# furkanyesiler/acoss

Measured on AMD Instinct MI355X. Metric: track-pairs/sec on N x N Serra09 Qmax (HPCP, T=2000), higher is better.
Workload: dtype f32

## Files before the change

acoss_amd/_lib.py:

```python
import ctypes
import os

import numpy as np

_HERE = os.path.dirname(os.path.abspath(__file__))
LIB_PATH = os.environ.get("ACX_LIB") or os.path.join(_HERE, "csrc", "libacx.so")

ACX_OK = 0
ACX_ERR_INVALID = -1
ACX_ERR_HIP = -2
ACX_ERR_NOMEM = -3
ACX_ERR_STATE = -4
ACX_ERR_SHORT = -5
ACX_ERR_UNSUPPORTED = -6

EXPORTS = [
    "acx_abi_version", "acx_create", "acx_destroy", "acx_last_error", "acx_set_scratch_limit",
    "acx_upload_pool", "acx_serra09_default_params", "acx_serra09_pairs", "acx_serra09_debug_pair",
    "acx_serra09_embed_len", "acx_profile_enable", "acx_profile_reset", "acx_profile_count",
    "acx_profile_get", "acx_debug_sqrt", "acx_debug_ef_sqrt", "acx_upload_pool_f64", "acx_simple_pairs",
    "acx_ef_upload_pool", "acx_earlyfusion_pairs", "acx_ef_debug_pair", "acx_sw_binary",
    "acx_chenfusion_pairs", "acx_csm_binary_sw", "acx_upload_raw_pool", "acx_download_pool",
    "acx_simple_upload_raw_pool", "acx_download_pool_f64", "acx_snf_fuse", "acx_qmax_binary",
    "acx_ef_block_features", "acx_ef_upload_raw_pool", "acx_snf_fuse_dists", "acx_grid_plan", "acx_pool_lengths", "acx_grid_run", "acx_grid_scatter", "acx_pair_grid",
    "acx_set_nonfinite_policy", "acx_nonfinite_zeroed", "acx_ef_pool_begin", "acx_ef_pool_tracks", "acx_ef_pool_end",
    "acx_set_ef_gemm", "acx_hip_versions",
    "acx_dev_alloc", "acx_dev_free", "acx_dev_read", "acx_dev_sync",
    "acx_comm_id", "acx_comm_init", "acx_comm_destroy", "acx_grid_allgather", "acx_pair_grid_ranks", "acx_set_ef_fuse",
    "acx_device_info", "acx_ef_debug_pairs",
    "acx_ftm2d_default_params", "acx_ftm2d_pool_begin", "acx_ftm2d_pool_tracks", "acx_ftm2d_pool_end",
    "acx_ftm2d_upload_shingles", "acx_ftm2d_download_shingles", "acx_ftm2d_debug_track", "acx_ftm2d_pairs",
    "acx_rank_columns", "acx_topk_rows",
    "acx_query_scores", "acx_query_topk", "acx_query_ranks", "acx_query_topk_lists",
    "acx_serra09_debug_bits", "acx_serra09_plan", "acx_serra09_family_name", "acx_serra09_fast_tail", "acx_serra09_fast_tail_launches",
    "acx_pool_append", "acx_pool_append_raw", "acx_pool_append_f64", "acx_ef_pool_append", "acx_ftm2d_append_shingles",
    "acx_pool_truncate",
    "acx_serra09_align", "acx_qmax_locate_binary",
    "acx_serra09_align_paths", "acx_qmax_path_binary",
    "acx_chenfusion_align", "acx_chenfusion_align_paths", "acx_dmax_locate_binary", "acx_dmax_path_binary",
    "acx_ef_debug_bits", "acx_csm_debug_bits", "acx_sw_bits_binary",
    "acx_ef_align", "acx_sw_align_binary",
    "acx_simple_profile",
    "acx_snf_debug_stages", "acx_snf_debug_update",
    "acx_ef_crossfusion_pairs", "acx_ef_crossfusion_debug", "acx_crossfusion_matrices", "acx_xsel_binary_sw",
    "acx_ef_download_pool",
]
ABI_VERSION = 4
COMM_ID_BYTES = 128

# ... 146 lines not shown
    L.acx_upload_pool.argtypes = [vp, fp, lp, ctypes.c_int32, ctypes.c_int32]
    L.acx_upload_raw_pool.argtypes = [vp, fp, lp, ctypes.c_int32, ctypes.c_int32, ctypes.c_int32, lp]
    L.acx_download_pool.argtypes = [vp, fp, ctypes.c_int64]
    L.acx_serra09_default_params.restype = None
    L.acx_serra09_default_params.argtypes = [pp]
    L.acx_serra09_pairs.argtypes = [vp, ip, ctypes.c_int64, pp, fp]
    L.acx_chenfusion_pairs.argtypes = [vp, ip, ctypes.c_int64, pp, fp]
    L.acx_serra09_debug_pair.argtypes = [vp, ctypes.c_int32, ctypes.c_int32, pp, fp, fp, fp, fp, fp, ip, fp, ip]
    L.acx_serra09_debug_bits.argtypes = [vp, ip, ctypes.c_int64, pp, fp, ctypes.POINTER(ctypes.c_uint8), ctypes.POINTER(ctypes.c_int64)]
    L.acx_serra09_plan.argtypes = [lp, ctypes.c_int32, ip, ctypes.c_int64, pp, ctypes.c_int64, ctypes.POINTER(Serra09PlanRec)]
    L.acx_serra09_family_name.restype = ctypes.c_char_p
    L.acx_serra09_family_name.argtypes = [ctypes.c_int32, ctypes.c_int32]
    L.acx_serra09_fast_tail.argtypes = [pp, ctypes.c_int32, ctypes.c_int32, ctypes.c_int32]
    L.acx_serra09_fast_tail_launches.restype = ctypes.c_int64
    L.acx_serra09_fast_tail_launches.argtypes = []
    L.acx_serra09_embed_len.restype = ctypes.c_int32
    L.acx_serra09_embed_len.argtypes = [ctypes.c_int32, pp]
    L.acx_profile_enable.argtypes = [vp, ctypes.c_int]
    L.acx_profile_reset.argtypes = [vp]
    L.acx_profile_count.argtypes = [vp]
    L.acx_profile_get.argtypes = [vp, ctypes.c_int, ctypes.c_char_p, ctypes.c_int,
                                  ctypes.POINTER(ctypes.c_double), lp, lp]
    L.acx_debug_sqrt.argtypes = [vp, fp, ctypes.c_int64, fp]
    L.acx_debug_ef_sqrt.argtypes = [vp, fp, ctypes.c_int64, fp]
    dp = ctypes.POINTER(ctypes.c_double)
    L.acx_upload_pool_f64.argtypes = [vp, dp, lp, ctypes.c_int32, ctypes.c_int32]
    L.acx_simple_upload_raw_pool.argtypes = [vp, fp, lp, ctypes.c_int32, ctypes.c_int32, ctypes.c_int32, ctypes.c_int32,
                                             ctypes.c_int32, lp]
    L.acx_download_pool_f64.argtypes = [vp, dp, ctypes.c_int64]
    L.acx_simple_pairs.argtypes = [vp, ip, ctypes.c_int64, ctypes.c_int32, ctypes.c_int32, dp]
# ... 180 lines not shown


def serra09_fast_tail(n_cells, role, params=None, debug=False):
    L = load()
    params = params if params is not None else serra09_params()
    rc = L.acx_serra09_fast_tail(ctypes.byref(params), int(n_cells), int(role), int(bool(debug)))
    if rc < 0:
        raise ValueError("acx_serra09_fast_tail: bad argument")
    return bool(rc)


def serra09_fast_tail_launches():
    return int(load().acx_serra09_fast_tail_launches())


def serra09_family_name(family, m):
    name = load().acx_serra09_family_name(int(family), int(m))
    if name is None:
        raise ValueError("unknown Serra09 kernel family %r" % (family,))
    return name.decode()


def grid_scatter(lengths, spec, gathered, rank_stride, planes, mirror, first=0, count=-1):
    L = load()
    lengths = np.ascontiguousarray(lengths, dtype=np.int64)
    gathered = np.ascontiguousarray(gathered, dtype=np.float32)
    n = len(lengths)
    for P in planes:
        if P.dtype != np.float32 or P.shape != (n, n) or not P.flags["C_CONTIGUOUS"]:
            raise ValueError("grid_scatter: planes must be C-contiguous (N, N) float32")
# ... 968 lines not shown
```

acoss_amd/csrc/acx.hip:

```cpp
#include <hip/hip_runtime.h>

#include <chrono>
#include <dlfcn.h>
#include <rccl/rccl.h>

#include <algorithm>
#include <cmath>
#include <cstdio>
#include <cstdlib>
#include <cstring>
#include <string>
#include <vector>

#include "../../include/acx.h"
#include "serra09_kernels.hpp"
#include "serra09_long_kernels.hpp"
#include "serra09_locate_kernels.hpp"
#include "serra09_path_kernels.hpp"
#include "chen_align_kernels.hpp"
#include "prep_kernels.hpp"
#include "snf_kernels.hpp"
#include "ef_crossfusion_kernels.hpp"
#include "simple_kernels.hpp"
#include "simple_profile_kernels.hpp"
// ... 56 lines not shown

struct acx_ctx {
    int device = 0;
    hipStream_t stream = nullptr;
    hipStream_t qstream = nullptr;
    hipStream_t qstream2 = nullptr;
    hipEvent_t q2_done = nullptr;
    std::string err;
    DeviceBuffer<float> d_frames0;
    DeviceBuffer<int64_t> d_toff0;
    std::vector<int64_t> h_off0;
    int pool_tau = 0;
    DeviceBuffer<float> d_frames;
    DeviceBuffer<float> d_frot;
    DeviceBuffer<_Float16> d_fh;
    DeviceBuffer<float> d_normtab;
    DeviceBuffer<int64_t> d_noff;
    int normtab_m = 0, normtab_span = -1;
    std::vector<int64_t> h_noff;
    DeviceBuffer<int64_t> d_toff;
    DeviceBuffer<float> d_gch;
    std::vector<int64_t> h_off;
    const float *active_frames() const { return d_frames ? d_frames.get() : d_frames0.get(); }
    const int64_t *active_toff() const { return d_toff ? d_toff.get() : d_toff0.get(); }
    int32_t n_tracks = 0, dim = 0;
    DeviceBuffer<double> d_frames64;
    DeviceBuffer<int64_t> d_toff64;
    DeviceBuffer<double> d_prof64;
    DeviceBuffer<double> d_wn64;
    int wn64_L = 0;
// ... 205 lines not shown
    if (p.pct_mode < 0 || p.pct_mode > 3) return fail(c, ACX_ERR_INVALID, "serra09: pct_mode must be 0..3");
    if (p.oti_target != 0 && p.oti_target != 1) return fail(c, ACX_ERR_INVALID, "serra09: oti_target must be 0 or 1");
    if (!(p.gamma_o >= 0.0f) || !(p.gamma_e >= 0.0f)) return fail(c, ACX_ERR_INVALID, "serra09: gammas must be >= 0");
    if (p.arith != ACX_ARITH_EXACT && p.arith != ACX_ARITH_F16X2) return fail(c, ACX_ERR_INVALID, "serra09: arith must be ACX_ARITH_EXACT or ACX_ARITH_F16X2");
    if (p.arith == ACX_ARITH_F16X2 && p.m != 9) return fail(c, ACX_ERR_UNSUPPORTED, "serra09: the f16x2 Gram exists for the default stack size m = 9 only");
    return ACX_OK;
}

constexpr int64_t POOL_SLACK = 96;

bool launch_band(acx_ctx *c, int m, const PairDesc *dpd, const std::vector<PairDesc> &hpd, int b0, int B, int maxRows, int cls,
                 const acx_serra09_params &p, int role, int write_d2, int want_eps)
{
    const float *operands = p.arith == ACX_ARITH_F16X2 ? reinterpret_cast<const float *>(c->d_fh + POOL_SLACK * acx::FH) : c->d_frot + POOL_SLACK * acx::FROT;
    acx::BandLaunch L{c->stream, operands, c->active_toff(), c->d_normtab + POOL_SLACK, c->d_noff, c->d_scratch, c->d_thr,
                      c->d_bits, p.kappa, p.pct_mode, p.inclusive, p.oti_target, 0};
    const int family = acx::serra09_band_family(cls, m, p.arith);
    bool ok = true;
    for (const acx::Serra09Run &r : acx::serra09_fast_tail_runs(p, family, role, write_d2 != 0, want_eps != 0, c->d_bits != nullptr, hpd, b0, b0 + B)) {
        L.fast_tail = r.fast ? 1 : 0;
        ok = ok && acx::launch_band_kernel(L, m, dpd + (r.begin - b0), r.end - r.begin, maxRows, family, role, write_d2, want_eps, p.arith);
    }
    return ok;
}

template <int M>
void launch_normtab(acx_ctx *c, int maxM, int span, int first, int count)
{
    hipLaunchKernelGGL((acx::normtab_kernel<M>), dim3(count, (maxM + 255) / 256, acx::NBIN), dim3(256), 0, c->stream,
                       c->active_frames(), c->active_toff() + first, c->d_noff + first, c->d_normtab + POOL_SLACK, span);
}
// ... 12 lines not shown
        case 13: CALL(13); break; case 14: CALL(14); break; case 15: CALL(15); break; case 16: CALL(16); break; \
        default: handled = false;                                                                   \
    }
#endif

int ensure_tau(acx_ctx *c, int tau)
{
    if (c->pool_tau == tau) return ACX_OK;
    c->normtab_m = 0; c->normtab_span = -1;
    c->pool_tau = 0;
    c->fh_base_n = -1;
    ACX_HIP(c, c->d_frames.reset());
    ACX_HIP(c, c->d_toff.reset());
    ACX_HIP(c, c->d_frot.reset());
    ACX_HIP(c, c->d_fh.reset());
    ACX_HIP(c, c->d_normtab.reset());
    ACX_HIP(c, c->d_noff.reset());
    const int n = c->n_tracks;
    DeviceBuffer<float> frames, frot;
    DeviceBuffer<int64_t> toff;
    if (tau == 1) {
        c->h_off = c->h_off0;
    } else {
        c->h_off.assign((size_t)n + 1, 0);
        int maxT = 1;
        for (int t = 0; t < n; ++t) {
            const int64_t T = c->h_off0[t + 1] - c->h_off0[t];
            const int64_t Td = (T + tau - 1) / tau;
            c->h_off[t + 1] = c->h_off[t] + Td;
            maxT = std::max<int>(maxT, (int)Td);
// ... 62 lines not shown
    DeviceBuffer<_Float16> fh;
    const hipError_t e = fh.grow(halfs);
    if (e != hipSuccess) return fail(c, ACX_ERR_NOMEM, std::string("serra09: the f16 operand pool does not fit the device: ") + hipGetErrorString(e));
    ACX_HIP(c, hipMemsetAsync(fh, 0, sizeof(_Float16) * halfs, c->stream));
    if (total > 0) {
        hipLaunchKernelGGL(acx::rotpool_f16_kernel, dim3((unsigned)std::min<int64_t>((total * 12 + 255) / 256, 1 << 22)), dim3(256), 0, c->stream,
                           c->active_frames(), fh + POOL_SLACK * acx::FH, total);
        ACX_HIP(c, hipGetLastError());
    }
    ACX_HIP(c, hipStreamSynchronize(c->stream));
    c->d_fh = std::move(fh);
    c->fh_base_n = total > 0 ? c->n_tracks : -1;
    return ACX_OK;
}

int ensure_normtab(acx_ctx *c, const acx_serra09_params &p)
{
    const int span = p.embed_full ? (p.m - 1) : p.m;
    if (c->d_normtab && c->normtab_m == p.m && c->normtab_span == span) return ACX_OK;
    ACX_HIP(c, c->d_normtab.reset());
    ACX_HIP(c, c->d_noff.reset());
    c->normtab_m = 0; c->normtab_span = -1;
    std::vector<int64_t> &noff = c->h_noff;
    noff.assign((size_t)c->n_tracks + 1, 0);
    int64_t tot = 0;
    int maxM = 1;
    for (int t = 0; t < c->n_tracks; ++t) {
        noff[t] = tot;
        const int Me = std::max<int>(0, (int)(c->h_off[t + 1] - c->h_off[t]) - span);
        maxM = std::max(maxM, Me);
// ... 17 lines not shown
    c->normtab_span = span;
    return ACX_OK;
}

struct DebugOut {
    float *d2, *epsq, *epsr, *thrq, *thrr;
    int32_t *oti;
    int32_t *dims;
};

int64_t scratch_limit_bytes(const acx_ctx *c)
{
    if (c->scratch_limit > 0) return c->scratch_limit;
    const char *env = getenv("ACX_SCRATCH_GB");
    if (env && atof(env) > 0) return (int64_t)(atof(env) * (double)(1ull << 30));
    return (int64_t)(0.40 * (double)c->total_mem);
}

int collect_slot(acx_ctx *c, Serra09Slot &s, float *out, acx_alignment *al = nullptr)
{
    if (!s.busy) return ACX_OK;
    ACX_HIP(c, hipEventSynchronize(s.done));
    for (int k2 = 0; s.al && al && k2 < s.B; ++k2) al[s.k0 + s.perm[k2]] = s.h_al[(size_t)k2];
    for (int k2 = 0; !s.al && out && k2 < s.B; ++k2)
        for (int e = 0; e < s.w; ++e) out[(size_t)s.w * (s.k0 + s.perm[k2]) + e] = s.h_out[(size_t)s.w * k2 + e];
    s.busy = false;
    drain_profile(c);
    return ACX_OK;
}

struct DevDst {
// ... 265 lines not shown

    int64_t k0 = 0;
    for (int batch = 0; k0 < K; ++batch) {
        Serra09Slot &S = c->slot[batch & 1];
        if ((rc = collect_slot(c, S, out, al)) != ACX_OK) return rc;
        std::vector<PairDesc> &pd = S.pd;
        acx::Serra09Arena used;
        const int64_t k = acx::serra09_pack_batch(len, pairs, k0, K, p, dbg != nullptr, limit_floats, pd, used);
        if (k == k0) return fail(c, ACX_ERR_STATE, "serra09: the batch plan made no progress at pair " + std::to_string(k0));
        const int B = (int)pd.size();
        const acx::Serra09Sort srt = acx::serra09_sort_batch(pd, S.sorted, S.perm, p.m);
        const int *key_begin = srt.key_begin, *cls_begin = srt.cls_begin;
        const std::vector<int> &perm = S.perm;
        if (cls_begin[NC] > 0 && (rc = ensure_normtab(c, p)) != ACX_OK) return rc;
        if (cls_begin[NC] > 0 && p.arith == ACX_ARITH_F16X2 && (rc = ensure_f16pool(c)) != ACX_OK) return rc;
        if ((rc = ensure(c, c->d_scratch, (size_t)std::max<int64_t>(used.scratch, 1))) != ACX_OK) return rc;
        if ((rc = ensure(c, c->d_bits, (size_t)std::max<int64_t>(used.bits, 1))) != ACX_OK) return rc;
        if ((rc = ensure(c, c->d_thr, (size_t)used.thr + 64 * 32 + 16)) != ACX_OK) return rc;
        if ((rc = ensure(c, S.d_pd, (size_t)B)) != ACX_OK) return rc;
        if ((rc = ensure(c, S.d_out, (size_t)2 * B)) != ACX_OK) return rc;
        if ((rc = ensure(c, S.h_out, (size_t)2 * B)) != ACX_OK) return rc;
        ACX_HIP(c, hipMemcpyAsync(S.d_pd, pd.data(), sizeof(PairDesc) * B, hipMemcpyHostToDevice, c->stream));
        if (al) {
            int64_t seams = 0;
            S.seam_off.resize((size_t)B);
            for (int k2 = 0; k2 < B; ++k2) { S.seam_off[(size_t)k2] = seams; seams += acx::loc_seam_records(pd[k2].Mq, pd[k2].Mr, p.dp_start); }
            if ((rc = ensure(c, S.d_al, (size_t)B)) != ACX_OK) return rc;
            if ((rc = ensure(c, S.h_al, (size_t)B)) != ACX_OK) return rc;
            if ((rc = ensure(c, S.d_seam_off, (size_t)B)) != ACX_OK) return rc;
            if ((rc = ensure(c, c->d_seam, (size_t)std::max<int64_t>(seams, 1))) != ACX_OK) return rc;
// ... 701 lines not shown
#undef ACX_ROWSTAT
#undef ACX_FUSESEL
#undef ACX_FUSESEL_K
#undef ACX_SW
    if (host_timing)
        fprintf(stderr, "[acx ef host] %lld pairs in %d batches, %.1f ms: preamble %.1f, descriptors %.1f, rectangles %.1f, enqueue %.1f, waiting for the device %.1f\n",
                (long long)K, nbatches, 1e3 * (now() - t_call), 1e3 * ht[4], 1e3 * ht[0], 1e3 * ht[1], 1e3 * ht[2], 1e3 * ht[3]);
    return ACX_OK;
}

static void free_pool(acx_ctx *c)
{
    for (DeviceBuffer<float> *b : {&c->d_frames0, &c->d_frames, &c->d_frot, &c->d_normtab, &c->d_gch}) (void)b->reset();
    for (DeviceBuffer<int64_t> *b : {&c->d_toff0, &c->d_toff, &c->d_noff}) (void)b->reset();
    (void)c->d_fh.reset();
    c->normtab_m = 0; c->normtab_span = -1;
    c->pool_tau = 0;
    c->fh_base_n = -1;
}

template <int L>
int launch_simple(acx_ctx *c, int n, size_t smem, int oti)
{
    auto kern = acx::simple_kernel<L>;
    int wpb = acx::SIMPLE_WPB;
    while (wpb > 1 && smem * wpb > 160 * 1024) --wpb;
    ACX_HIP(c, hipFuncSetAttribute(reinterpret_cast<const void *>(kern), hipFuncAttributeMaxDynamicSharedMemorySize, (int)(smem * wpb)));
    hipLaunchKernelGGL(kern, dim3((n + wpb - 1) / wpb), dim3(64 * wpb), smem * wpb, c->stream, c->d_frames64, c->d_toff64,
                       c->d_prof64, c->d_wn64, c->d_pairs, c->d_out64, oti, n, (int)smem);
    return ACX_OK;
// ... 2590 lines not shown
    return ACX_OK;
}

struct S09Tail {
    int n0 = 0, n1 = 0;
    std::vector<int64_t> off0, aoff, noff;
    int maxT = 1, maxM = 1;
    bool active = false, table = false;
};

static int s09_append_begin(acx_ctx *c, const char *who, const int64_t *rel, int32_t n_new, S09Tail &t)
{
    quiesce(c);
    const int dim = c->dim, tau = c->pool_tau;
    t.n0 = c->n_tracks; t.n1 = t.n0 + n_new;
    const int64_t total0 = c->h_off0[t.n0], total1 = total0 + rel[n_new];
    t.active = dim == acx::NBIN && tau >= 1 && c->d_frames0 && c->d_toff0;
    t.table = t.active && c->d_normtab && c->d_noff && c->normtab_m > 0;
    const int64_t atotal0 = t.active ? c->h_off[t.n0] : 0, tot0 = t.table ? c->h_noff[t.n0] : 0;
    t.off0.resize((size_t)n_new + 1); t.aoff.assign((size_t)n_new + 1, atotal0); t.noff.assign((size_t)n_new + 1, tot0);
    for (int i = 0; i <= n_new; ++i) t.off0[i] = total0 + rel[i];
    for (int i = 0; i < n_new && t.active; ++i) {
        const int64_t T = rel[i + 1] - rel[i], Ta = tau == 1 ? T : (T + tau - 1) / tau;
        if (Ta > 0x7fffffffLL) return fail(c, ACX_ERR_INVALID, std::string(who) + ": offsets: a track has more than 2^31 - 1 frames");
        t.aoff[i + 1] = t.aoff[i] + Ta;
        t.maxT = std::max<int>(t.maxT, (int)Ta);
        if (t.table) {
            const int Me = std::max<int>(0, (int)Ta - c->normtab_span);
            t.maxM = std::max(t.maxM, Me);
            t.noff[i + 1] = t.noff[i] + (int64_t)acx::NBIN * (Me + acx::NGUARD);
// ... 172 lines not shown
    if (rc != ACX_OK) return rc;
    if ((rc = s09_append_finish(c, t)) != ACX_OK) return rc;
    if (pooled_offsets_out) memcpy(pooled_offsets_out, poff.data(), sizeof(int64_t) * (n_new + 1));
    return ACX_OK;
}

static int s09_truncate(acx_ctx *c, int32_t n)
{
    quiesce(c);
    const bool table = c->d_normtab && c->normtab_m > 0 && c->pool_tau >= 1;
    const int64_t norm_hi = table ? c->h_noff[c->n_tracks] : 0;
    c->n_tracks = n;
    c->h_off0.resize((size_t)n + 1);
    if (c->pool_tau >= 1) c->h_off.resize((size_t)n + 1);
    if (table) c->h_noff.resize((size_t)n + 1);
    if (c->d_fh && (c->fh_base_n < 0 || n < c->fh_base_n)) {
        ACX_HIP(c, c->d_fh.reset());
        c->fh_base_n = -1;
    }
    plan_forget(c);
    return s09_seal(c, norm_hi);
}


int acx_pool_append_f64(acx_ctx *c, const double *frames, const int64_t *offsets, int32_t n_new, int32_t dim)
{
    if (!c) return ACX_ERR_INVALID;
    if (!c->d_frames64) return fail(c, ACX_ERR_STATE, "pool_append_f64: f64 feature pool not uploaded (acx_upload_pool_f64)");
    if (!offsets) return fail(c, ACX_ERR_INVALID, "pool_append_f64: offsets must not be NULL");
    int rc;
// ... 256 lines not shown
                r.batch = batch;
                r.cr = cl; r.cq = band ? acx::serra09_row_class(pd[k2].Mq) : acx::SERRA09_NC;
                r.row_family = band ? acx::serra09_band_family(r.cr, params->m, params->arith) : ACX_SERRA09_FAMILY_STREAMING;
                r.col_family = band ? acx::serra09_band_family(r.cq, params->m, params->arith) : ACX_SERRA09_FAMILY_STREAMING;
                r.sweep_cols = sw.cols; r.sweep_pack = sw.pack;
            }
        }
        k0 = k;
    }
    return ACX_OK;
}

const char *acx_serra09_family_name(int32_t family, int32_t m) { return acx::serra09_family_name(family, m); }

int64_t acx_serra09_fast_tail_launches(void) { return (int64_t)acx::fast_tail_launches(); }

int acx_serra09_fast_tail(const acx_serra09_params *params, int32_t n_cells, int32_t role, int32_t debug)
{
    if (!params || n_cells < 1 || check_params(nullptr, *params) != ACX_OK) return ACX_ERR_INVALID;
    const int cl = acx::serra09_row_class(n_cells);
    if (cl >= acx::SERRA09_NC || params->m > acx::MAX_M) return 0;
    const bool dbg = debug != 0;
    return acx::serra09_fast_tail_params(*params, acx::serra09_band_family(cl, params->m, params->arith), role, dbg && role == 0, dbg, true) &&
           acx::serra09_fast_tail_row(acx::pct_position(n_cells, params->kappa, params->pct_mode), n_cells) ? 1 : 0;
}

int acx_pool_lengths(acx_ctx *c, int32_t algo, int64_t *lengths, int32_t capacity, int32_t *n_tracks)
{
    if (!c) return ACX_ERR_INVALID;
    std::vector<int64_t> len;
// ... 1007 lines not shown
```

acoss_amd/csrc/acx_band.hip:

```cpp
#include <hip/hip_runtime.h>

#include <atomic>
#include <cassert>

#include "serra09_kernels.hpp"
#include "serra09_band2_kernels.hpp"
#include "serra09_plan.hpp"

namespace acx {

namespace {

std::atomic<long long> g_fast_tail_launches{0};

template <int M>
bool launch_band_m(const BandLaunch &L, const PairDesc *dpd, int B, int maxRows, int family, int role, int write_d2, int want_eps, int arith)
{
    const dim3 grid((maxRows + BAND - 1) / BAND, B, 1);
#define ACX_BAND_K(V4_, R_, W_, A_, F_) hipLaunchKernelGGL((band_kernel<M, V4_, R_, W_, A_, F_>), grid, dim3(BAND_THREADS), 0, L.stream, \
                                                  L.frot, L.toff, L.normtab, L.noff, dpd, L.scratch, L.thr, L.bits, L.kappa, \
                                                  L.pct_mode, L.inclusive, L.oti_target, want_eps)
#define ACX_BAND_A(V4_, A_) do { if (role) ACX_BAND_K(V4_, 1, false, A_, false); else if (write_d2) ACX_BAND_K(V4_, 0, true, A_, false); else ACX_BAND_K(V4_, 0, false, A_, false); } while (0)
    if (L.fast_tail) {
        assert(family == ACX_SERRA09_FAMILY_BAND_8 && arith == ACX_ARITH_EXACT && !write_d2 && !want_eps);
        if (role) ACX_BAND_K(8, 1, false, 0, true); else ACX_BAND_K(8, 0, false, 0, true);
        g_fast_tail_launches.fetch_add(1, std::memory_order_relaxed);
        return true;
    }
#define ACX_BAND(V4_) do { if (arith == ACX_ARITH_EXACT) ACX_BAND_A(V4_, 0); else if constexpr (M == 9) ACX_BAND_A(V4_, 1); else return false; return true; } while (0)
#define ACX_BAND2_K(R_, W_, NV_, GL_) hipLaunchKernelGGL((band2_kernel<M, R_, W_, NV_, GL_>), grid, dim3(64 * B2Geom<NV_, GL_>::WAVES), 0, L.stream, L.frot, L.normtab, \
                                                         dpd, L.scratch, L.thr, L.bits, L.pct_mode, L.inclusive, L.oti_target, want_eps)
#define ACX_BAND2(NV_, GL_) do { if constexpr (M <= 9) { if (arith != ACX_ARITH_EXACT) return false; \
                                     if (role) ACX_BAND2_K(1, false, NV_, GL_); else if (write_d2) ACX_BAND2_K(0, true, NV_, GL_); else ACX_BAND2_K(0, false, NV_, GL_); \
                                     return true; } return false; } while (0)
    if (arith != ACX_ARITH_EXACT && arith != ACX_ARITH_F16X2) return false;
    switch (family) {
    case ACX_SERRA09_FAMILY_BAND2_4ROWS: ACX_BAND2(B2_NV, 16);
    case ACX_SERRA09_FAMILY_BAND2_2ROWS: ACX_BAND2(B2_NV, 32);
    case ACX_SERRA09_FAMILY_BAND2_MID: ACX_BAND2(B2_NV_MID, 32);
    case ACX_SERRA09_FAMILY_BAND_2: ACX_BAND(2);
    case ACX_SERRA09_FAMILY_BAND_4: ACX_BAND(4);
    case ACX_SERRA09_FAMILY_BAND_8: ACX_BAND(8);
    }
    return false;
#undef ACX_BAND2
#undef ACX_BAND2_K
#undef ACX_BAND
#undef ACX_BAND_A
#undef ACX_BAND_K
}

}

bool launch_band_kernel(const BandLaunch &L, int m, const PairDesc *dpd, int B, int maxRows, int family, int role, int write_d2, int want_eps, int arith)
{
    switch (m) {
#define ACX_CASE(M_) case M_: return launch_band_m<M_>(L, dpd, B, maxRows, family, role, write_d2, want_eps, arith);
#ifdef ACX_FAST_BUILD
#ifndef ACX_FAST_BUILD_M
#define ACX_FAST_BUILD_M 9
#endif
        ACX_CASE(ACX_FAST_BUILD_M)
#else
        ACX_CASE(1) ACX_CASE(2) ACX_CASE(3) ACX_CASE(4) ACX_CASE(5) ACX_CASE(6) ACX_CASE(7) ACX_CASE(8)
        ACX_CASE(9) ACX_CASE(10) ACX_CASE(11) ACX_CASE(12) ACX_CASE(13) ACX_CASE(14) ACX_CASE(15) ACX_CASE(16)
#endif
#undef ACX_CASE
    }
    return false;
}

long long fast_tail_launches() { return g_fast_tail_launches.load(std::memory_order_relaxed); }

}

#ifdef ACX_TIMING
extern "C" int acx_dev_band_timing(unsigned long long *out, int reset)
{
    if (hipDeviceSynchronize() != hipSuccess) return -1;
    if (hipMemcpyFromSymbol(out, HIP_SYMBOL(acx::g_band_clk), sizeof(unsigned long long) * 32) != hipSuccess) return -1;
    if (reset) {
        unsigned long long z[32] = {0};
        if (hipMemcpyToSymbol(HIP_SYMBOL(acx::g_band_clk), z, sizeof(z)) != hipSuccess) return -1;
    }
    return 0;
}
#endif
// ... 1 lines not shown
```

acoss_amd/csrc/serra09_kernels.hpp:

```cpp
#pragma once
#include <hip/hip_runtime.h>
#include <stdint.h>
#include <type_traits>

namespace acx {

constexpr int NBIN = 12;
constexpr int SEL_BINS = 2048;
constexpr int MAX_M = 16;
constexpr int NGUARD = 80;

struct PctPos { float kf, fl, ce; int32_t ilo, ihi, k; };
__host__ __device__ inline PctPos pct_position(int n, float kappa, int pct_mode)
{
    PctPos p;
    p.kf = (n > 1) ? (float)(n - 1) * kappa : (float)n * kappa;
    p.fl = floorf(p.kf); p.ce = ceilf(p.kf);
    int ilo = (int)p.fl, ihi = (int)p.ce;
    ilo = ilo < 0 ? 0 : (ilo > n - 1 ? n - 1 : ilo);
    ihi = ihi < 0 ? 0 : (ihi > n - 1 ? n - 1 : ihi);
    int k = ilo;
    if (pct_mode == 3) {
        k = (int)floorf(p.kf + 0.5f);
        k = k > n - 1 ? n - 1 : k;
// ... 706 lines not shown
constexpr int BAND = 8;
constexpr int BAND_THREADS = 512;
constexpr int FROT = 3 * NBIN;

static __global__ void rotpool_kernel(const float *__restrict__ pool, float *__restrict__ frot, int64_t nframes)
{
    const int64_t total = nframes * FROT, stride = (int64_t)gridDim.x * blockDim.x;
    for (int64_t idx = (int64_t)blockIdx.x * blockDim.x + threadIdx.x; idx < total; idx += stride) {
        const int64_t f = idx / FROT;
        const int e = (int)(idx - f * FROT);
        const int r = e / NBIN, rem = e - r * NBIN, cls = rem / 3, kb = rem - 3 * cls;
        frot[idx] = pool[f * NBIN + cls + 4 * ((r + kb) % 3)];
    }
}

constexpr int FH = 12 * 8;
static __global__ void rotpool_f16_kernel(const float *__restrict__ pool, _Float16 *__restrict__ fh, int64_t nframes)
{
    const int64_t total = nframes * 12, stride = (int64_t)gridDim.x * blockDim.x;
    for (int64_t idx = (int64_t)blockIdx.x * blockDim.x + threadIdx.x; idx < total; idx += stride) {
        const int64_t f = idx / 12;
        const int e = (int)(idx - f * 12), r = e >> 2, cls = e & 3;
        _Float16 h1[3], h2[3];
#pragma unroll
        for (int j = 0; j < 3; ++j) {
            const float x = pool[f * NBIN + cls + 4 * ((r + j) % 3)];
            h1[j] = (_Float16)x;
            h2[j] = (_Float16)(x - (float)h1[j]);
        }
        _Float16 *o = fh + idx * 8;
// ... 11 lines not shown
    if (e >= n) return;
    const int t = e / NBIN, b = e - t * NBIN;
    out[o0 * NBIN + e] = in[(toff_in[track] + (int64_t)t * tau) * NBIN + b];
}

struct BandLaunch {
    hipStream_t stream;
    const float *frot;
    const int64_t *toff;
    const float *normtab;
    const int64_t *noff;
    float *scratch, *thr;
    unsigned long long *bits;
    float kappa;
    int pct_mode, inclusive, oti_target;
    int fast_tail;
};
bool launch_band_kernel(const BandLaunch &L, int m, const struct PairDesc *dpd, int B, int maxRows, int family, int role,
                        int write_d2, int want_eps, int arith);
long long fast_tail_launches();

#ifdef ACX_ABL
#define ACX_ABL_EXIT(n_, val_) do { if (ACX_ABL == (n_)) { if ((val_) == 1.2345e-30f) thr[0] = 1.0f; return; } } while (0)
#else
#define ACX_ABL_EXIT(n_, val_) do { } while (0)
#endif

#ifdef ACX_TIMING
__device__ unsigned long long g_band_clk[32];
struct StampT { unsigned long long t; int base; };
#define ACX_STAMP(slot) do { const unsigned long long now_ = __builtin_readcyclecounter(); \
        if (lane == 0) atomicAdd(&g_band_clk[tstamp_.base + (slot)], now_ - tstamp_.t); tstamp_.t = now_; } while (0)
#else
#define ACX_STAMP(slot) do { } while (0)
#endif
// ... 196 lines not shown
    float thr_row;
    if (SNAP && inclusive && dlo <= eps && eps < dhi) thr_row = slo;
    else thr_row = d2_threshold(eps, inclusive);
    ACX_STAMP(6);
    float *X = thr + P.offX;
    if (lane == 0) {
        const int o = role ? P.pitchT + row : row;
        X[o] = thr_row;
        X[P.pitchT + P.pitchD + o] = eps;
    }
    band_row_bits<NV, ROLE, TC_VIA_LDS, FAST>(xr, tcg, thr_row, myrow, lane, row, MB, cshift, P, thr, bits);
    ACX_STAMP(7);
}

constexpr int band_waves_per_simd(int m, int v4, int arith = 0) { return (v4 <= 2 && m <= 9) ? ACX_NARROW_WAVES : ((v4 <= 4 && m <= 9) ? (arith ? 6 : ACX_MID_WAVES) : 4); }
template <int M, int V4, int ROLE, bool WD2 = false, int ARITH = 0, bool FAST = false>
__global__ __launch_bounds__(BAND_THREADS, band_waves_per_simd(M, V4, ARITH)) void band_kernel(const float *__restrict__ frot,
                                                            const int64_t *__restrict__ toff,
                                                            const float *__restrict__ normtab,
                                                            const int64_t *__restrict__ noff,
                                                            const PairDesc *__restrict__ pd,
                                                            float *__restrict__ scratch,
                                                            float *__restrict__ thr,
                                                            unsigned long long *__restrict__ bits,
                                                            float kappa, int pct_mode, int inclusive, int oti_target, int want_eps)
{
    constexpr bool write_d2 = WD2;
    static_assert(!FAST || (V4 == 8 && ARITH == 0 && !WD2), "the product-path tail exists for the wide class of the exact arithmetic");
    using G = BandGeom<M, V4, ARITH>;
    constexpr int role = ROLE;
    constexpr int NV = 4 * V4;
    constexpr int NSTEP = NV / 8;
    using RG = RowGeom<NV>;
    constexpr int LNP = RG::LNP, ROWP = RG::ROWP, FBINS = RG::FBINS;
    constexpr bool HIST_IN_ROW = RG::HIST_IN_ROW;
    constexpr int SWEEP_FLOATS = 8 * G::AROWS * G::SP;
    constexpr int LDS_FLOATS = SWEEP_FLOATS > RG::TAIL_FLOATS ? SWEEP_FLOATS : RG::TAIL_FLOATS;
    __shared__ __attribute__((aligned(4096))) float smem[LDS_FLOATS];

    const int bid_x = blockIdx.x, bid_y = blockIdx.y;
    const PairDesc P = pd[bid_y];
    const int MA = role ? P.Mr : P.Mq, MB = role ? P.Mq : P.Mr;
    const int TA = role ? P.Tr : P.Tq, TB = role ? P.Tq : P.Tr;
    const int i0 = bid_x * BAND;
    if (i0 >= MA) return;
    const int tid = threadIdx.x, lane = tid & 63;
    const int wave = __builtin_amdgcn_readfirstlane(tid >> 6);
    const bool rows_are_ref = role == 1;
    const int rota = (rows_are_ref == (oti_target == 0)) ? P.oti : 0;
    const int rotb = (rows_are_ref == (oti_target == 0)) ? 0 : P.oti;
    const float *nrow = normtab + (role ? P.nr : P.nq) + (int64_t)rota * (MA + NGUARD);
    const float *ncol = normtab + (role ? P.nq : P.nr) + (int64_t)rotb * (MB + NGUARD);
    const float INF = __builtin_inff();
    const float PADV = INF;

    const int lr = lane & 15, lk = lane >> 4;
    int c0a = lk - rota; if (c0a < 0) c0a += NBIN;
    int c0b = lk - rotb; if (c0b < 0) c0b += NBIN;
    constexpr unsigned PB = ARITH ? (unsigned)FH * 2u : (unsigned)FROT * 4u;
    const unsigned offA = ARITH ? (unsigned)(((c0a >> 2) * 4 + (c0a & 3)) * 16) : (unsigned)(((c0a >> 2) * NBIN + (c0a & 3) * 3) * 4);
    const unsigned offB = ARITH ? (unsigned)(((c0b >> 2) * 4 + (c0b & 3)) * 16) : (unsigned)(((c0b >> 2) * NBIN + (c0b & 3) * 3) * 4);
    const char *pool_b = reinterpret_cast<const char *>(frot);
    const char *fra = pool_b + (role ? P.fr : P.fq) * (int64_t)PB + offA;
    const __amdgpu_buffer_rsrc_t rsB =
        __builtin_amdgcn_make_buffer_rsrc((void *)(pool_b + ((role ? P.fq : P.fr) - 8) * (int64_t)PB), 0, -1, 0x00020000);
    const unsigned voffB = offB + (unsigned)lr * PB;
    const char *frb = pool_b + (role ? P.fq : P.fr) * (int64_t)PB + offB;
    typedef float f32x3 __attribute__((ext_vector_type(3)));
    typedef f32x3 f32x3_u __attribute__((aligned(4)));
    typedef unsigned u32x3 __attribute__((ext_vector_type(3)));
    typedef u32x3 u32x3_u __attribute__((aligned(4)));
    typedef unsigned u32x4v __attribute__((ext_vector_type(4)));
    typedef _Float16 f16x8 __attribute__((ext_vector_type(8)));
    typedef _Float16 f16x4 __attribute__((ext_vector_type(4)));
    float areg[G::NRT][3];
    f16x8 ah8[G::NRT], ah9[G::NRT];
#pragma unroll
    for (int ta = 0; ta < G::NRT; ++ta) {
        int f = i0 + 16 * ta + lr;
        f = f > TA - 1 ? TA - 1 : f;
        if constexpr (ARITH == 0) {
            const f32x3 v = *reinterpret_cast<const f32x3_u *>(fra + (size_t)f * PB);
            areg[ta][0] = v.x; areg[ta][1] = v.y; areg[ta][2] = v.z;
        } else {
            const u32x3 w = *reinterpret_cast<const u32x3_u *>(fra + (size_t)f * PB);
            const u32x4v a = {w.x, (w.y & 0xffffu) | (w.x << 16), (w.x >> 16) | (w.y << 16), (w.y >> 16) | (w.z << 16)};
            const u32x4v a9 = {(w.z >> 16) | (w.y & 0xffff0000u), w.z, 0u, 0u};
            ah8[ta] = __builtin_bit_cast(f16x8, a);
            ah9[ta] = __builtin_bit_cast(f16x8, a9);
        }
    }
    float xrow[BAND];
#pragma unroll
    for (int a = 0; a < BAND; ++a) xrow[a] = (i0 + a < MA) ? nrow[i0 + a] : INF;
    float *Sw = smem + wave * (G::AROWS * G::SP);
    const PctPos pp = role ? P.pos_q : P.pos_r;
#ifdef ACX_TIMING
    StampT tstamp_{__builtin_readcyclecounter(), 0};
    if (lane == 0) atomicAdd(&g_band_clk[15], 1ull);
#endif

    const int ntiles = (MB + BAND - 1 + 63) / 64;
    typedef unsigned BvT[G::NCT][ARITH ? 4 : 3];
    typedef f32x4 AccT[G::NRT][G::NCT];
    auto load_operands = [&](int tile, BvT &bv, auto tb0_tag) {
        constexpr int tb0 = decltype(tb0_tag)::value;
        const int base = 64 * tile - (BAND - 1);
        if constexpr (V4 >= 8) {
            const unsigned so = (unsigned)(base + 8) * PB;
#pragma unroll
            for (int tb = tb0; tb < G::NCT; ++tb) {
                if constexpr (ARITH == 0) {
                    const u32x3 v = __builtin_amdgcn_raw_buffer_load_b96(rsB, voffB, so + 16u * PB * tb, 0);
                    bv[tb][0] = v.x; bv[tb][1] = v.y; bv[tb][2] = v.z;
                } else {
                    const u32x4v v = __builtin_amdgcn_raw_buffer_load_b128(rsB, voffB, so + 16u * PB * tb, 0);
                    bv[tb][0] = v.x; bv[tb][1] = v.y; bv[tb][2] = v.z; bv[tb][3] = v.w;
                }
            }
        } else {
            const char *p = frb + (ptrdiff_t)(base + lr) * (ptrdiff_t)PB;
#pragma unroll
            for (int tb = tb0; tb < G::NCT; ++tb) {
                if constexpr (ARITH == 0) {
                    const u32x3 v = *reinterpret_cast<const u32x3_u *>(p + 16 * PB * tb);
                    bv[tb][0] = v.x; bv[tb][1] = v.y; bv[tb][2] = v.z;
                } else {
                    const u32x4v v = *reinterpret_cast<const u32x4v *>(p + 16 * PB * tb);
// ... 554 lines not shown
```

acoss_amd/csrc/serra09_plan.hpp:

```cpp
#pragma once
#include <algorithm>
#include <cstdint>
#include <cstdlib>
#include <vector>

#include "../../include/acx.h"
#include "serra09_kernels.hpp"

namespace acx {

inline int serra09_tiles(int M) { return (M + BAND - 1 + 63) / 64; }

inline int64_t serra09_round_up(int64_t v, int64_t m) { return (v + m - 1) / m * m; }

inline int serra09_embed_len(int T, int m, int tau, int embed_full)
{
    const int span = embed_full ? (m - 1) * tau : m * tau;
    const int L = T - span;
    if (L <= 0) return 0;
    return (L + tau - 1) / tau;
}

constexpr int SERRA09_NC = 5;
struct Serra09Class {
// ... 7 lines not shown
    {12, ACX_SERRA09_FAMILY_BAND2_MID, ACX_SERRA09_FAMILY_BAND_4, ACX_SERRA09_FAMILY_BAND_4, 16, 1},
    {16, ACX_SERRA09_FAMILY_BAND_4, ACX_SERRA09_FAMILY_BAND_4, ACX_SERRA09_FAMILY_BAND_4, 16, 1},
    {32, ACX_SERRA09_FAMILY_BAND_8, ACX_SERRA09_FAMILY_BAND_8, ACX_SERRA09_FAMILY_BAND_8, 32, 1},
};

inline int serra09_row_class(int M)
{
    const int nd = serra09_tiles(M);
    int cl = 0;
    while (cl < SERRA09_NC && nd > SERRA09_CLASS[cl].tiles) ++cl;
    return cl;
}

struct Serra09Switches {
    int band2;
    bool multi, qstream;
};
inline const Serra09Switches &serra09_switches()
{
    static const Serra09Switches s = [] {
        auto off = [](const char *name) { const char *e = getenv(name); return e && e[0] == '0'; };
        const char *b = getenv("ACX_BAND2");
        return Serra09Switches{(b && b[0] >= '0' && b[0] <= '2') ? b[0] - '0' : 3, !off("ACX_QMAX_MULTI"), !off("ACX_QMAX_STREAM")};
    }();
    return s;
}

inline int serra09_band_family(int cl, int m, int arith)
{
    const Serra09Class &c = SERRA09_CLASS[cl];
    if (arith == ACX_ARITH_F16X2) return c.band_f16;
    if (m > 9) return c.band_m10;
    const int keep = serra09_switches().band2;
    switch (c.band_m9) {
    case ACX_SERRA09_FAMILY_BAND2_4ROWS: return keep >= 3 ? c.band_m9 : (keep >= 1 ? ACX_SERRA09_FAMILY_BAND2_2ROWS : ACX_SERRA09_FAMILY_BAND_2);
    case ACX_SERRA09_FAMILY_BAND2_2ROWS: return keep >= 1 ? c.band_m9 : ACX_SERRA09_FAMILY_BAND_2;
    case ACX_SERRA09_FAMILY_BAND2_MID: return keep >= 2 ? c.band_m9 : ACX_SERRA09_FAMILY_BAND_4;
    default: return c.band_m9;
// ... 178 lines not shown
```

include/acx.h:

```cpp
#ifndef ACX_H
#define ACX_H

#include <stdint.h>

#ifdef __cplusplus
extern "C" {
#endif

#define ACX_ABI_VERSION 4

enum {
    ACX_OK = 0,
    ACX_ERR_INVALID = -1,
    ACX_ERR_HIP = -2,
    ACX_ERR_NOMEM = -3,
    ACX_ERR_STATE = -4,
    ACX_ERR_SHORT = -5,
    ACX_ERR_UNSUPPORTED = -6
};

typedef struct acx_ctx acx_ctx;


acx_ctx *acx_create(int device, int *err);
// ... 91 lines not shown
    ACX_SERRA09_FAMILY_BAND_8 = 5,
    ACX_SERRA09_FAMILY_STREAMING = 6
};
typedef struct acx_serra09_plan_rec {
    int32_t Mq, Mr;
    int32_t batch;
    int32_t cr, cq;
    int32_t row_family, col_family;
    int32_t sweep_cols, sweep_pack;
} acx_serra09_plan_rec;
int acx_serra09_plan(const int64_t *lengths, int32_t n_tracks, const int32_t *pairs, int64_t K,
                     const acx_serra09_params *params, int64_t scratch_limit, acx_serra09_plan_rec *out);
const char *acx_serra09_family_name(int32_t family, int32_t m);
int acx_serra09_fast_tail(const acx_serra09_params *params, int32_t n_cells, int32_t role, int32_t debug);
int64_t acx_serra09_fast_tail_launches(void);


int acx_upload_pool_f64(acx_ctx *ctx, const double *frames, const int64_t *offsets,
                        int32_t n_tracks, int32_t dim);

int acx_simple_upload_raw_pool(acx_ctx *ctx, const float *raw, const int64_t *raw_offsets, int32_t n_tracks,
                               int32_t dim, int32_t win, int32_t skip, int32_t win_len_smooth,
                               int64_t *pooled_offsets_out);

int acx_download_pool_f64(acx_ctx *ctx, double *frames, int64_t capacity);

int acx_simple_pairs(acx_ctx *ctx, const int32_t *pairs, int64_t K, int32_t sslen, int32_t oti,
                     double *out);

typedef struct {
// ... 236 lines not shown
```

Baseline: 109,100.

## Precompute per-rotation operand planes for the wide exact-arithmetic band kernel

Adds a device buffer holding, for each of the 12 chroma rotations, a contiguous per-frame copy of the rotated pool. The wide (V4=8, exact) band kernel then loads its column operands from the plane matching the column rotation with a fixed lane offset, instead of computing per-lane rotated offsets into the shared rotated pool. It also moves a few scalar loads and the early exit around with asm barriers, and drops the per-row bounds check by reading guard entries. The cost is 12x extra device memory for the pool, a one-time build kernel, invalidation whenever the pool changes, and a smaller scratch budget.

```diff
diff --git a/acoss_amd/_lib.py b/acoss_amd/_lib.py
--- a/acoss_amd/_lib.py
+++ b/acoss_amd/_lib.py
@@ -33,6 +33,7 @@
     "acx_rank_columns", "acx_topk_rows",
     "acx_query_scores", "acx_query_topk", "acx_query_ranks", "acx_query_topk_lists",
     "acx_serra09_debug_bits", "acx_serra09_plan", "acx_serra09_family_name", "acx_serra09_fast_tail", "acx_serra09_fast_tail_launches",
+    "acx_serra09_plane_launches",
     "acx_pool_append", "acx_pool_append_raw", "acx_pool_append_f64", "acx_ef_pool_append", "acx_ftm2d_append_shingles",
     "acx_pool_truncate",
     "acx_serra09_align", "acx_qmax_locate_binary",
@@ -209,6 +210,8 @@
     L.acx_serra09_fast_tail.argtypes = [pp, ctypes.c_int32, ctypes.c_int32, ctypes.c_int32]
     L.acx_serra09_fast_tail_launches.restype = ctypes.c_int64
     L.acx_serra09_fast_tail_launches.argtypes = []
+    L.acx_serra09_plane_launches.restype = ctypes.c_int64
+    L.acx_serra09_plane_launches.argtypes = []
     L.acx_serra09_embed_len.restype = ctypes.c_int32
     L.acx_serra09_embed_len.argtypes = [ctypes.c_int32, pp]
     L.acx_profile_enable.argtypes = [vp, ctypes.c_int]
@@ -419,6 +422,10 @@
     return int(load().acx_serra09_fast_tail_launches())
 
 
+def serra09_plane_launches():
+    return int(load().acx_serra09_plane_launches())
+
+
 def serra09_family_name(family, m):
     name = load().acx_serra09_family_name(int(family), int(m))
     if name is None:
diff --git a/acoss_amd/csrc/acx.hip b/acoss_amd/csrc/acx.hip
--- a/acoss_amd/csrc/acx.hip
+++ b/acoss_amd/csrc/acx.hip
@@ -94,6 +94,8 @@
     DeviceBuffer<float> d_frames;
     DeviceBuffer<float> d_frot;
     DeviceBuffer<_Float16> d_fh;
+    DeviceBuffer<float> d_planes;
+    int64_t plane_floats = 0;
     DeviceBuffer<float> d_normtab;
     DeviceBuffer<int64_t> d_noff;
     int normtab_m = 0, normtab_span = -1;
@@ -329,7 +331,8 @@
 {
     const float *operands = p.arith == ACX_ARITH_F16X2 ? reinterpret_cast<const float *>(c->d_fh + POOL_SLACK * acx::FH) : c->d_frot + POOL_SLACK * acx::FROT;
     acx::BandLaunch L{c->stream, operands, c->active_toff(), c->d_normtab + POOL_SLACK, c->d_noff, c->d_scratch, c->d_thr,
-                      c->d_bits, p.kappa, p.pct_mode, p.inclusive, p.oti_target, 0};
+                      c->d_bits, p.kappa, p.pct_mode, p.inclusive, p.oti_target,
+                      c->d_planes ? c->d_planes + POOL_SLACK * acx::FPLANE : nullptr, c->plane_floats, 0};
     const int family = acx::serra09_band_family(cls, m, p.arith);
     bool ok = true;
     for (const acx::Serra09Run &r : acx::serra09_fast_tail_runs(p, family, role, write_d2 != 0, want_eps != 0, c->d_bits != nullptr, hpd, b0, b0 + B)) {
@@ -372,6 +375,7 @@
     ACX_HIP(c, c->d_toff.reset());
     ACX_HIP(c, c->d_frot.reset());
     ACX_HIP(c, c->d_fh.reset());
+    ACX_HIP(c, c->d_planes.reset());
     ACX_HIP(c, c->d_normtab.reset());
     ACX_HIP(c, c->d_noff.reset());
     const int n = c->n_tracks;
@@ -464,6 +468,29 @@
     return ACX_OK;
 }
 
+int ensure_planes(acx_ctx *c)
+{
+    if (c->d_planes || !acx::serra09_switches().planes) return ACX_OK;
+    const int64_t total = c->h_off[c->n_tracks];
+    const int64_t plane_floats = (std::max<int64_t>(1, total) + 2 * POOL_SLACK) * acx::FPLANE;
+    DeviceBuffer<float> planes;
+    const hipError_t e = planes.grow((size_t)plane_floats * acx::NBIN);
+    if (e != hipSuccess)
+        return fail(c, ACX_ERR_NOMEM, std::string("serra09: the wide class's operand planes (576 bytes per pooled frame) do not fit the device: ") +
+                                          hipGetErrorString(e) + "; ACX_PLANES=0 runs that class from the rotated pool");
+    ACX_HIP(c, hipMemsetAsync(planes, 0, sizeof(float) * (size_t)plane_floats * acx::NBIN, c->stream));
+    if (total > 0) {
+        const int64_t nout = total * acx::FPLANE * acx::NBIN;
+        hipLaunchKernelGGL(acx::planepool_kernel, dim3((unsigned)std::min<int64_t>((nout + 255) / 256, 1 << 22)), dim3(256), 0, c->stream,
+                           c->d_frot + POOL_SLACK * acx::FROT, planes + POOL_SLACK * acx::FPLANE, total, plane_floats);
+        ACX_HIP(c, hipGetLastError());
+    }
+    ACX_HIP(c, hipStreamSynchronize(c->stream));
+    c->d_planes = std::move(planes);
+    c->plane_floats = plane_floats;
+    return ACX_OK;
+}
+
 int ensure_normtab(acx_ctx *c, const acx_serra09_params &p)
 {
     const int span = p.embed_full ? (p.m - 1) : p.m;
@@ -511,7 +538,7 @@
     if (c->scratch_limit > 0) return c->scratch_limit;
     const char *env = getenv("ACX_SCRATCH_GB");
     if (env && atof(env) > 0) return (int64_t)(atof(env) * (double)(1ull << 30));
-    return (int64_t)(0.40 * (double)c->total_mem);
+    return (int64_t)(0.40 * (double)(c->total_mem - (int64_t)(c->d_planes.capacity() * sizeof(float))));
 }
 
 int collect_slot(acx_ctx *c, Serra09Slot &s, float *out, acx_alignment *al = nullptr)
@@ -807,6 +834,11 @@
         const std::vector<int> &perm = S.perm;
         if (cls_begin[NC] > 0 && (rc = ensure_normtab(c, p)) != ACX_OK) return rc;
         if (cls_begin[NC] > 0 && p.arith == ACX_ARITH_F16X2 && (rc = ensure_f16pool(c)) != ACX_OK) return rc;
+        {
+            bool wide = cls_begin[NC] > cls_begin[NC - 1];
+            for (int cl = 0; cl < NC; ++cl) wide = wide || key_begin[NC * cl + NC] > key_begin[NC * cl + NC - 1];
+            if (wide && p.arith == ACX_ARITH_EXACT && (rc = ensure_planes(c)) != ACX_OK) return rc;
+        }
         if ((rc = ensure(c, c->d_scratch, (size_t)std::max<int64_t>(used.scratch, 1))) != ACX_OK) return rc;
         if ((rc = ensure(c, c->d_bits, (size_t)std::max<int64_t>(used.bits, 1))) != ACX_OK) return rc;
         if ((rc = ensure(c, c->d_thr, (size_t)used.thr + 64 * 32 + 16)) != ACX_OK) return rc;
@@ -1538,6 +1570,7 @@
     for (DeviceBuffer<float> *b : {&c->d_frames0, &c->d_frames, &c->d_frot, &c->d_normtab, &c->d_gch}) (void)b->reset();
     for (DeviceBuffer<int64_t> *b : {&c->d_toff0, &c->d_toff, &c->d_noff}) (void)b->reset();
     (void)c->d_fh.reset();
+    (void)c->d_planes.reset();
     c->normtab_m = 0; c->normtab_span = -1;
     c->pool_tau = 0;
     c->fh_base_n = -1;
@@ -4158,6 +4191,7 @@
     quiesce(c);
     const int dim = c->dim, tau = c->pool_tau;
     t.n0 = c->n_tracks; t.n1 = t.n0 + n_new;
+    ACX_HIP(c, c->d_planes.reset());
     const int64_t total0 = c->h_off0[t.n0], total1 = total0 + rel[n_new];
     t.active = dim == acx::NBIN && tau >= 1 && c->d_frames0 && c->d_toff0;
     t.table = t.active && c->d_normtab && c->d_noff && c->normtab_m > 0;
@@ -4360,6 +4394,7 @@
     c->h_off0.resize((size_t)n + 1);
     if (c->pool_tau >= 1) c->h_off.resize((size_t)n + 1);
     if (table) c->h_noff.resize((size_t)n + 1);
+    ACX_HIP(c, c->d_planes.reset());
     if (c->d_fh && (c->fh_base_n < 0 || n < c->fh_base_n)) {
         ACX_HIP(c, c->d_fh.reset());
         c->fh_base_n = -1;
@@ -4646,6 +4681,7 @@
 const char *acx_serra09_family_name(int32_t family, int32_t m) { return acx::serra09_family_name(family, m); }
 
 int64_t acx_serra09_fast_tail_launches(void) { return (int64_t)acx::fast_tail_launches(); }
+int64_t acx_serra09_plane_launches(void) { return (int64_t)acx::plane_launches(); }
 
 int acx_serra09_fast_tail(const acx_serra09_params *params, int32_t n_cells, int32_t role, int32_t debug)
 {
diff --git a/acoss_amd/csrc/acx_band.hip b/acoss_amd/csrc/acx_band.hip
--- a/acoss_amd/csrc/acx_band.hip
+++ b/acoss_amd/csrc/acx_band.hip
@@ -12,14 +12,19 @@
 namespace {
 
 std::atomic<long long> g_fast_tail_launches{0};
+std::atomic<long long> g_plane_launches{0};
 
 template <int M>
 bool launch_band_m(const BandLaunch &L, const PairDesc *dpd, int B, int maxRows, int family, int role, int write_d2, int want_eps, int arith)
 {
     const dim3 grid((maxRows + BAND - 1) / BAND, B, 1);
-#define ACX_BAND_K(V4_, R_, W_, A_, F_) hipLaunchKernelGGL((band_kernel<M, V4_, R_, W_, A_, F_>), grid, dim3(BAND_THREADS), 0, L.stream, \
+#define ACX_BAND_KP(V4_, R_, W_, A_, F_, P_) hipLaunchKernelGGL((band_kernel<M, V4_, R_, W_, A_, F_, P_>), grid, dim3(BAND_THREADS), 0, L.stream, \
                                                   L.frot, L.toff, L.normtab, L.noff, dpd, L.scratch, L.thr, L.bits, L.kappa, \
-                                                  L.pct_mode, L.inclusive, L.oti_target, want_eps)
+                                                  L.pct_mode, L.inclusive, L.oti_target, want_eps, L.planes, L.plane_floats)
+#define ACX_BAND_K(V4_, R_, W_, A_, F_) do { if constexpr (V4_ == 8 && A_ == 0) { \
+                                                 if (L.planes) { ACX_BAND_KP(V4_, R_, W_, A_, F_, true); g_plane_launches.fetch_add(1, std::memory_order_relaxed); } \
+                                                 else ACX_BAND_KP(V4_, R_, W_, A_, F_, false); } \
+                                             else ACX_BAND_KP(V4_, R_, W_, A_, F_, false); } while (0)
 #define ACX_BAND_A(V4_, A_) do { if (role) ACX_BAND_K(V4_, 1, false, A_, false); else if (write_d2) ACX_BAND_K(V4_, 0, true, A_, false); else ACX_BAND_K(V4_, 0, false, A_, false); } while (0)
     if (L.fast_tail) {
         assert(family == ACX_SERRA09_FAMILY_BAND_8 && arith == ACX_ARITH_EXACT && !write_d2 && !want_eps);
@@ -48,6 +53,7 @@
 #undef ACX_BAND
 #undef ACX_BAND_A
 #undef ACX_BAND_K
+#undef ACX_BAND_KP
 }
 
 }
@@ -71,6 +77,7 @@
 }
 
 long long fast_tail_launches() { return g_fast_tail_launches.load(std::memory_order_relaxed); }
+long long plane_launches() { return g_plane_launches.load(std::memory_order_relaxed); }
 
 }
 
diff --git a/acoss_amd/csrc/serra09_kernels.hpp b/acoss_amd/csrc/serra09_kernels.hpp
--- a/acoss_amd/csrc/serra09_kernels.hpp
+++ b/acoss_amd/csrc/serra09_kernels.hpp
@@ -744,6 +744,24 @@
     }
 }
 
+constexpr int FPLANE = NBIN;
+__host__ __device__ constexpr int plane_src(int rot, int e)
+{
+    const int lk = e / 3, kb = e - 3 * lk;
+    const int c0 = (lk - rot + NBIN) % NBIN;
+    return (c0 >> 2) * NBIN + (c0 & 3) * 3 + kb;
+}
+static __global__ void planepool_kernel(const float *__restrict__ frot, float *__restrict__ planes, int64_t nframes, int64_t plane_floats)
+{
+    const int64_t per = nframes * FPLANE, total = per * NBIN, stride = (int64_t)gridDim.x * blockDim.x;
+    for (int64_t idx = (int64_t)blockIdx.x * blockDim.x + threadIdx.x; idx < total; idx += stride) {
+        const int rot = (int)(idx / per);
+        const int64_t w = idx - rot * per, f = w / FPLANE;
+        const int e = (int)(w - f * FPLANE);
+        planes[rot * plane_floats + w] = frot[f * FROT + plane_src(rot, e)];
+    }
+}
+
 constexpr int FH = 12 * 8;
 static __global__ void rotpool_f16_kernel(const float *__restrict__ pool, _Float16 *__restrict__ fh, int64_t nframes)
 {
@@ -785,11 +803,14 @@
     unsigned long long *bits;
     float kappa;
     int pct_mode, inclusive, oti_target;
+    const float *planes;
+    int64_t plane_floats;
     int fast_tail;
 };
 bool launch_band_kernel(const BandLaunch &L, int m, const struct PairDesc *dpd, int B, int maxRows, int family, int role,
                         int write_d2, int want_eps, int arith);
 long long fast_tail_launches();
+long long plane_launches();
 
 #ifdef ACX_ABL
 #define ACX_ABL_EXIT(n_, val_) do { if (ACX_ABL == (n_)) { if ((val_) == 1.2345e-30f) thr[0] = 1.0f; return; } } while (0)
@@ -1016,7 +1037,7 @@
 }
 
 constexpr int band_waves_per_simd(int m, int v4, int arith = 0) { return (v4 <= 2 && m <= 9) ? ACX_NARROW_WAVES : ((v4 <= 4 && m <= 9) ? (arith ? 6 : ACX_MID_WAVES) : 4); }
-template <int M, int V4, int ROLE, bool WD2 = false, int ARITH = 0, bool FAST = false>
+template <int M, int V4, int ROLE, bool WD2 = false, int ARITH = 0, bool FAST = false, bool PLANES = false>
 __global__ __launch_bounds__(BAND_THREADS, band_waves_per_simd(M, V4, ARITH)) void band_kernel(const float *__restrict__ frot,
                                                             const int64_t *__restrict__ toff,
                                                             const float *__restrict__ normtab,
@@ -1025,9 +1046,11 @@
                                                             float *__restrict__ scratch,
                                                             float *__restrict__ thr,
                                                             unsigned long long *__restrict__ bits,
-                                                            float kappa, int pct_mode, int inclusive, int oti_target, int want_eps)
+                                                            float kappa, int pct_mode, int inclusive, int oti_target, int want_eps,
+                                                            const float *__restrict__ planes, int64_t plane_floats)
 {
     constexpr bool write_d2 = WD2;
+    static_assert(!PLANES || (V4 == 8 && ARITH == 0), "the operand planes exist for the wide class of the exact arithmetic");
     static_assert(!FAST || (V4 == 8 && ARITH == 0 && !WD2), "the product-path tail exists for the wide class of the exact arithmetic");
     using G = BandGeom<M, V4, ARITH>;
     constexpr int role = ROLE;
@@ -1041,11 +1064,16 @@
     __shared__ __attribute__((aligned(4096))) float smem[LDS_FLOATS];
 
     const int bid_x = blockIdx.x, bid_y = blockIdx.y;
-    const PairDesc P = pd[bid_y];
+    constexpr bool EAGER_HEAD = V4 == 8 && ARITH == 0;
+    int pd_idx = bid_y;
+    if constexpr (EAGER_HEAD) asm("" : "+s"(pd_idx) : "s"(frot), "s"(normtab), "s"(oti_target), "s"(planes), "s"(plane_floats));
+    const PairDesc P = pd[pd_idx];
     const int MA = role ? P.Mr : P.Mq, MB = role ? P.Mq : P.Mr;
     const int TA = role ? P.Tr : P.Tq, TB = role ? P.Tq : P.Tr;
     const int i0 = bid_x * BAND;
-    if (i0 >= MA) return;
+    int ma_exit = MA;
+    if constexpr (EAGER_HEAD) asm("" : "+s"(ma_exit) : "s"(P.Tq), "s"(P.Tr), "s"(P.Mq), "s"(P.Mr), "s"(P.oti), "s"(P.fq), "s"(P.fr), "s"(P.nq), "s"(P.nr));
+    if (i0 >= ma_exit) return;
     const int tid = threadIdx.x, lane = tid & 63;
     const int wave = __builtin_amdgcn_readfirstlane(tid >> 6);
     const bool rows_are_ref = role == 1;
@@ -1060,13 +1088,15 @@
     int c0a = lk - rota; if (c0a < 0) c0a += NBIN;
     int c0b = lk - rotb; if (c0b < 0) c0b += NBIN;
     constexpr unsigned PB = ARITH ? (unsigned)FH * 2u : (unsigned)FROT * 4u;
+    constexpr unsigned PBB = PLANES ? (unsigned)FPLANE * 4u : PB;
     const unsigned offA = ARITH ? (unsigned)(((c0a >> 2) * 4 + (c0a & 3)) * 16) : (unsigned)(((c0a >> 2) * NBIN + (c0a & 3) * 3) * 4);
     const unsigned offB = ARITH ? (unsigned)(((c0b >> 2) * 4 + (c0b & 3)) * 16) : (unsigned)(((c0b >> 2) * NBIN + (c0b & 3) * 3) * 4);
     const char *pool_b = reinterpret_cast<const char *>(frot);
     const char *fra = pool_b + (role ? P.fr : P.fq) * (int64_t)PB + offA;
+    const char *col_b = PLANES ? reinterpret_cast<const char *>(planes + rotb * plane_floats) : pool_b;
     const __amdgpu_buffer_rsrc_t rsB =
-        __builtin_amdgcn_make_buffer_rsrc((void *)(pool_b + ((role ? P.fq : P.fr) - 8) * (int64_t)PB), 0, -1, 0x00020000);
-    const unsigned voffB = offB + (unsigned)lr * PB;
+        __builtin_amdgcn_make_buffer_rsrc((void *)(col_b + ((role ? P.fq : P.fr) - 8) * (int64_t)PBB), 0, -1, 0x00020000);
+    const unsigned voffB = (PLANES ? 12u * (unsigned)lk : offB) + (unsigned)lr * PBB;
     const char *frb = pool_b + (role ? P.fq : P.fr) * (int64_t)PB + offB;
     typedef float f32x3 __attribute__((ext_vector_type(3)));
     typedef f32x3 f32x3_u __attribute__((aligned(4)));
@@ -1094,7 +1124,11 @@
     }
     float xrow[BAND];
 #pragma unroll
-    for (int a = 0; a < BAND; ++a) xrow[a] = (i0 + a < MA) ? nrow[i0 + a] : INF;
+    for (int a = 0; a < BAND; ++a) {
+        if constexpr (EAGER_HEAD) xrow[a] = nrow[i0 + a];
+        else xrow[a] = (i0 + a < MA) ? nrow[i0 + a] : INF;
+    }
+    static_assert(BAND - 1 <= NGUARD, "the band's rows past the matrix read guard entries");
     float *Sw = smem + wave * (G::AROWS * G::SP);
     const PctPos pp = role ? P.pos_q : P.pos_r;
 #ifdef ACX_TIMING
@@ -1109,11 +1143,11 @@
         constexpr int tb0 = decltype(tb0_tag)::value;
         const int base = 64 * tile - (BAND - 1);
         if constexpr (V4 >= 8) {
-            const unsigned so = (unsigned)(base + 8) * PB;
+            const unsigned so = (unsigned)(base + 8) * PBB;
 #pragma unroll
             for (int tb = tb0; tb < G::NCT; ++tb) {
                 if constexpr (ARITH == 0) {
-                    const u32x3 v = __builtin_amdgcn_raw_buffer_load_b96(rsB, voffB, so + 16u * PB * tb, 0);
+                    const u32x3 v = __builtin_amdgcn_raw_buffer_load_b96(rsB, voffB, so + 16u * PBB * tb, 0);
                     bv[tb][0] = v.x; bv[tb][1] = v.y; bv[tb][2] = v.z;
                 } else {
                     const u32x4v v = __builtin_amdgcn_raw_buffer_load_b128(rsB, voffB, so + 16u * PB * tb, 0);
diff --git a/acoss_amd/csrc/serra09_plan.hpp b/acoss_amd/csrc/serra09_plan.hpp
--- a/acoss_amd/csrc/serra09_plan.hpp
+++ b/acoss_amd/csrc/serra09_plan.hpp
@@ -45,14 +45,14 @@
 
 struct Serra09Switches {
     int band2;
-    bool multi, qstream;
+    bool multi, qstream, planes;
 };
 inline const Serra09Switches &serra09_switches()
 {
     static const Serra09Switches s = [] {
         auto off = [](const char *name) { const char *e = getenv(name); return e && e[0] == '0'; };
         const char *b = getenv("ACX_BAND2");
-        return Serra09Switches{(b && b[0] >= '0' && b[0] <= '2') ? b[0] - '0' : 3, !off("ACX_QMAX_MULTI"), !off("ACX_QMAX_STREAM")};
+        return Serra09Switches{(b && b[0] >= '0' && b[0] <= '2') ? b[0] - '0' : 3, !off("ACX_QMAX_MULTI"), !off("ACX_QMAX_STREAM"), !off("ACX_PLANES")};
     }();
     return s;
 }
diff --git a/include/acx.h b/include/acx.h
--- a/include/acx.h
+++ b/include/acx.h
@@ -129,6 +129,7 @@
 const char *acx_serra09_family_name(int32_t family, int32_t m);
 int acx_serra09_fast_tail(const acx_serra09_params *params, int32_t n_cells, int32_t role, int32_t debug);
 int64_t acx_serra09_fast_tail_launches(void);
+int64_t acx_serra09_plane_launches(void);
 
 
 int acx_upload_pool_f64(acx_ctx *ctx, const double *frames, const int64_t *offsets,
```

Result: faster. 112,100 (median of 6 runs) (+2.7%).
